# AshishKumar4/FlaxDiff

Measured on AMD Instinct MI355X. Metric: train images/sec/node (64x64 uncond EDM UNet, bs=256), higher is better.
Workload: dtype bf16; 1 GPU; model=unet_64px_[64,128,256,512]_res2_heads4, global_batch=256, resolution=64, parallelism=dp1, schedule=EDM + KarrasPredictionTransform(sigma_data=0.5)

## Files before the change

flaxdiff_amd/ops/hip/bindings.cpp:

```cpp
#include <torch/extension.h>
#include <tuple>
#include <vector>

std::vector<torch::Tensor> gn_silu_fwd(torch::Tensor x, torch::Tensor gamma,
                                       torch::Tensor beta, long groups,
                                       double eps, bool silu,
                                       c10::optional<torch::Tensor> x_b);
std::vector<torch::Tensor> gn_silu_bwd(torch::Tensor dy, torch::Tensor x,
                                       torch::Tensor gamma, torch::Tensor beta,
                                       torch::Tensor mean, torch::Tensor rstd,
                                       long groups, bool silu,
                                       c10::optional<torch::Tensor> dgamma_sink,
                                       c10::optional<torch::Tensor> dbeta_sink,
                                       c10::optional<torch::Tensor> add,
                                       c10::optional<torch::Tensor> x_b);
std::vector<torch::Tensor> rms_norm_fwd(torch::Tensor x, torch::Tensor gamma,
                                        double eps);
std::vector<torch::Tensor> rms_norm_bwd(torch::Tensor dy, torch::Tensor x,
                                        torch::Tensor gamma, torch::Tensor rrms,
                                        c10::optional<torch::Tensor> dgamma_sink);
torch::Tensor conv2d_fwd(torch::Tensor x, torch::Tensor w, torch::Tensor bias,
                         long stride, torch::Tensor add, torch::Tensor badd);
torch::Tensor conv2d_fwd_up2x(torch::Tensor x, torch::Tensor w,
                              torch::Tensor bias);
// ... 18 lines not shown
                                            torch::Tensor lse, double scale);
std::vector<torch::Tensor> attn_bwd_smallkv_v2(torch::Tensor q, torch::Tensor k,
                                               torch::Tensor v, torch::Tensor dout,
                                               torch::Tensor lse, double scale);
std::vector<torch::Tensor> attn_bwd_stream(torch::Tensor q, torch::Tensor k,
                                           torch::Tensor v, torch::Tensor o,
                                           torch::Tensor dout, torch::Tensor lse,
                                           double scale);
std::vector<int64_t> attn_bwd_stream_geometry(int64_t D);
torch::Tensor fwd_diffusion(torch::Tensor x0, torch::Tensor eps,
                            torch::Tensor a, torch::Tensor s);
torch::Tensor upsample2x_fwd(torch::Tensor x);
torch::Tensor time_embed(torch::Tensor t, torch::Tensor freqs, long features,
                         double max_positions);
torch::Tensor upsample2x_bwd(torch::Tensor dy);
torch::Tensor colsum(torch::Tensor x, c10::optional<torch::Tensor> sink);
torch::Tensor cat2_lastdim(torch::Tensor a, torch::Tensor b);
std::vector<torch::Tensor> split2_lastdim(torch::Tensor dy, long Ca, long Cb);
torch::Tensor geglu_fwd(torch::Tensor h);
torch::Tensor geglu_bwd(torch::Tensor dy, torch::Tensor h);
torch::Tensor wl2_loss_fwd(torch::Tensor pred, torch::Tensor target,
                           torch::Tensor wb);
torch::Tensor wl2_loss_bwd(torch::Tensor pred, torch::Tensor target,
                           torch::Tensor wb, torch::Tensor go);
torch::Tensor s5_scan_fwd(torch::Tensor a, torch::Tensor bu);
std::vector<torch::Tensor> s5_scan_bwd(torch::Tensor a, torch::Tensor x,
                                       torch::Tensor dx);
torch::Tensor gemm_fwd(torch::Tensor x, torch::Tensor w, torch::Tensor bias);
torch::Tensor gemm_dx(torch::Tensor dy, torch::Tensor w);
torch::Tensor gemm_nt(torch::Tensor x, torch::Tensor wt, torch::Tensor bias,
// ... 37 lines not shown
    m.def("attn_fwd", &attn_fwd, "flash attention forward (bf16, fp32 softmax)");
    m.def("attn_bwd_smallkv", &attn_bwd_smallkv,
          "fused attention backward for Skv<=128, D<=32");
    m.def("attn_bwd_smallkv_v2", &attn_bwd_smallkv_v2,
          "vectorized-LDS attention backward for Skv<=128, D<=64");
    m.def("attn_bwd_stream", &attn_bwd_stream,
          "key-streaming attention backward for any Sq/Skv, D<=128",
          py::arg("q"), py::arg("k"), py::arg("v"), py::arg("o"),
          py::arg("dout"), py::arg("lse"), py::arg("scale"));
    m.def("attn_bwd_stream_geometry", &attn_bwd_stream_geometry,
          "(DP, KB, QS) of attn_bwd_stream at head dim D");
    m.def("fwd_diffusion", &fwd_diffusion, "forward-diffusion axpy");
    m.def("upsample2x_fwd", &upsample2x_fwd, "nearest 2x upsample");
    m.def("time_embed", &time_embed, "fused sinusoidal/Fourier time embedding");
    m.def("upsample2x_bwd", &upsample2x_bwd, "nearest 2x upsample backward");
    m.def("colsum", &colsum, "coalesced column sum (bias grads)",
          py::arg("x"), py::arg("sink") = py::none());
    m.def("cat2_lastdim", &cat2_lastdim, "fused last-dim 2-tensor concat");
    m.def("split2_lastdim", &split2_lastdim, "one-pass last-dim split (cat backward)");
    m.def("geglu_fwd", &geglu_fwd, "fused GEGLU forward");
    m.def("geglu_bwd", &geglu_bwd, "fused GEGLU backward");
    m.def("wl2_loss_fwd", &wl2_loss_fwd, "fused weighted L2 loss forward");
    m.def("wl2_loss_bwd", &wl2_loss_bwd, "fused weighted L2 loss backward");
    m.def("s5_scan_fwd", &s5_scan_fwd, "S5 diagonal scan forward");
    m.def("s5_scan_bwd", &s5_scan_bwd, "S5 diagonal scan backward");
    m.def("gemm_fwd", &gemm_fwd, "MFMA bf16 GEMM y = x@w (+bias)");
    m.def("gemm_dx", &gemm_dx, "MFMA bf16 GEMM dx = dy@w^T");
    m.def("gemm_nt", &gemm_nt, "MFMA bf16 GEMM y = x@wt^T (+bias)",
          py::arg("x"), py::arg("wt"), py::arg("bias"), py::arg("add"),
          py::arg("x2") = py::none());
// ... 5 lines not shown
```

flaxdiff_amd/ops/hip/common.h:

```cpp
#pragma once

#include <hip/hip_runtime.h>
#include <hip/hip_bf16.h>
#include <hip/hip_fp16.h>
#include <cstdint>
#include <cstdlib>

#define FD_WAVE 64

__device__ __forceinline__ float bf2f(ushort u) {
    union { uint32_t i; float f; } c;
    c.i = uint32_t(u) << 16;
    return c.f;
}

__device__ __forceinline__ ushort f2bf(float f) {
    union { float f; uint32_t i; } c;
    c.f = f;
    uint32_t x = c.i;
    uint32_t lsb = (x >> 16) & 1;
    x += 0x7fff + lsb;
    return ushort(x >> 16);
}

typedef ushort ushort8 __attribute__((ext_vector_type(8)));
typedef float float8 __attribute__((ext_vector_type(8)));
typedef short bf16x8 __attribute__((ext_vector_type(8)));
typedef short bf16x4 __attribute__((ext_vector_type(4)));
typedef float f32x4 __attribute__((ext_vector_type(4)));
typedef float f32x16 __attribute__((ext_vector_type(16)));

struct BF16Tag {};
struct F32Tag {};

template <typename T> struct ElemIO;
template <> struct ElemIO<ushort> {
    static __device__ __forceinline__ float ld(const ushort* p) { return bf2f(*p); }
// ... 108 lines not shown
```

flaxdiff_amd/ops/hip/elementwise.hip:

```cpp
#include <torch/extension.h>
#include <ATen/hip/HIPContext.h>
#include "common.h"
#include "host_util.h"

template <typename T>
__global__ void fwd_diffusion_kernel(const T* __restrict__ x0,
                                     const T* __restrict__ eps,
                                     const float* __restrict__ a,
                                     const float* __restrict__ s,
                                     T* __restrict__ y,
                                     long per_sample, long total) {
    long i0 = (long)(blockIdx.x) * blockDim.x + threadIdx.x;
    const long stride = (long)gridDim.x * blockDim.x;
    for (long i = i0; i < total; i += stride) {
        const long b = i / per_sample;
        const float av = a[b], sv = s[b];
        ElemIO<T>::st(y + i, av * ElemIO<T>::ld(x0 + i) + sv * ElemIO<T>::ld(eps + i));
    }
}

template <typename T>
__global__ void upsample2x_fwd_kernel(const T* __restrict__ x, T* __restrict__ y,
                                      int H, int W, int C, long total_out) {
    long i0 = (long)(blockIdx.x) * blockDim.x + threadIdx.x;
// ... 139 lines not shown
    auto out = torch::empty({B, F}, tf.options());
    const float* fptr = nullptr;
    torch::Tensor ff;
    if (freqs.defined() && freqs.numel()) {
        ff = freqs.to(at::kFloat).contiguous();
        fptr = ff.data_ptr<float>();
    }
    const long total = (long)B * (F / 2);
    auto stream = at::hip::getCurrentHIPStream();
    hipLaunchKernelGGL(time_embed_kernel,
                       dim3((unsigned)((total + 255) / 256)), dim3(256), 0,
                       stream, tf.data_ptr<float>(), fptr,
                       out.data_ptr<float>(), B, F, (float)max_positions);
    FD_CHECK_LAUNCH();
    return out;
}


union GNV8_E { uint4 q; ushort u[8]; };

__global__ void colsum_kernel(const ushort* __restrict__ x,
                              float* __restrict__ out,
                              const long M, const int C,
                              const int rows_per_block) {
    extern __shared__ float csm[];
    const long r0 = (long)blockIdx.x * rows_per_block;
    const long r1 = min(r0 + rows_per_block, M);
    const int tpr = C >> 3;
    const int nsub = blockDim.x / tpr;
    for (int c = threadIdx.x; c < C; c += blockDim.x) csm[c] = 0.f;
// ... 338 lines not shown
```

flaxdiff_amd/ops/hip/gn_silu.hip:

```cpp
#include <torch/extension.h>
#include <ATen/hip/HIPContext.h>
#include "common.h"
#include "host_util.h"

template <typename T, bool SILU>
__global__ void gn_silu_fwd_kernel(const T* __restrict__ x,
                                   const float* __restrict__ gamma,
                                   const float* __restrict__ beta,
                                   T* __restrict__ y,
                                   float* __restrict__ mean_out,
                                   float* __restrict__ rstd_out,
                                   int S, int C, int G, float eps) {
    const int b = blockIdx.x / G;
    const int g = blockIdx.x % G;
    const int Cg = C / G;
    const long base = (long)b * S * C + (long)g * Cg;
    const long n = (long)S * Cg;

    __shared__ float scratch[4];

    float s1 = 0.f, s2 = 0.f;
    for (long i = threadIdx.x; i < n; i += blockDim.x) {
        const int s = i / Cg, c = i % Cg;
        const float v = ElemIO<T>::ld(x + base + (long)s * C + c);
// ... 90 lines not shown
            float dxv = rstd * (dz * gam - (s1 + xn * s2) * inv_n);
            if (HAS_ADD) dxv += ElemIO<T>::ld(add + idx);
            ElemIO<T>::st(dx + idx, dxv);
        }
        atomicAdd(dg_loc + c, dg_p);
        atomicAdd(db_loc + c, db_p);
    }

    __syncthreads();
    for (int cc = threadIdx.x; cc < Cg; cc += blockDim.x) {
        atomicAdd(dgamma + g * Cg + cc, dg_loc[cc]);
        atomicAdd(dbeta + g * Cg + cc, db_loc[cc]);
    }
}

union GNV8 { uint4 q; ushort u[8]; };



#define GN3_NTH 256

template <bool DUAL, typename P>
__device__ __forceinline__ P* gn3_src(P* xa, P* xb, const long row,
                                      const int c8, const int C, const int Ca) {
    if (DUAL)
        return c8 < Ca ? xa + row * Ca + c8 : xb + row * (C - Ca) + (c8 - Ca);
    return xa + row * C + c8;
}

template <bool SILU, bool DUAL = false>
__global__ void gn3_fwd_stats_kernel(const ushort* __restrict__ x,
                                     float* __restrict__ sums,
                                     const int S, const int C, const int G,
                                     const int Cg, const int chunk_rows,
                                     const FastDiv fdCg,
                                     const ushort* __restrict__ xb,
                                     const int Ca) {
    extern __shared__ float sm[];
    const int b = blockIdx.x;
    const int s0 = blockIdx.y * chunk_rows;
    const int s1lim = min(s0 + chunk_rows, S);
    const int tpr = C >> 3;
    const int nsub = GN3_NTH / tpr;
    const bool active = (int)threadIdx.x < nsub * tpr && nsub > 0;
    const int c8 = (threadIdx.x % tpr) * 8;
    const int srow = threadIdx.x / tpr;
    for (int i = threadIdx.x; i < 2 * G; i += GN3_NTH) sm[i] = 0.f;
    __syncthreads();

    float a1 = 0.f, a2 = 0.f;
    if (active) {
        for (int s = s0 + srow; s < s1lim; s += nsub) {
            GNV8 pk;
            pk.q = *reinterpret_cast<const uint4*>(
                gn3_src<DUAL>(x, xb, (long)b * S + s, c8, C, Ca));
            #pragma unroll
            for (int j = 0; j < 8; ++j) {
                const float v = bf2f(pk.u[j]);
                a1 += v; a2 += v * v;
            }
        }
        const int g = (int)fd_div((unsigned)c8, fdCg);
        atomicAdd(sm + g * 2 + 0, a1);
        atomicAdd(sm + g * 2 + 1, a2);
    }
    __syncthreads();
    for (int i = threadIdx.x; i < 2 * G; i += GN3_NTH)
        if (sm[i] != 0.f) atomicAdd(sums + (long)b * 2 * G + i, sm[i]);
}

template <bool SILU, bool DUAL = false>
__global__ void gn3_fwd_apply_kernel(const ushort* __restrict__ x,
                                     const float* __restrict__ sums,
                                     const float* __restrict__ gamma,
                                     const float* __restrict__ beta,
                                     ushort* __restrict__ y,
                                     float* __restrict__ mean_out,
                                     float* __restrict__ rstd_out,
                                     const int S, const int C, const int G,
                                     const int Cg, const int chunk_rows,
                                     const float eps, const FastDiv fdCg,
                                     const ushort* __restrict__ xb,
                                     const int Ca) {
    extern __shared__ float sm[];
    float* mr = sm;
    float* gam = sm + 2 * G;
    float* bet = gam + C;
    const int b = blockIdx.x;
    const int s0 = blockIdx.y * chunk_rows;
    const int s1lim = min(s0 + chunk_rows, S);
    const long base = ((long)b * S + s0) * C;
    const long n = (long)(s1lim - s0) * C;
    const float inv_n = 1.f / ((long)S * Cg);
    for (int g = threadIdx.x; g < G; g += GN3_NTH) {
        const float m = sums[(long)b * 2 * G + g * 2 + 0] * inv_n;
        const float var = fmaxf(sums[(long)b * 2 * G + g * 2 + 1] * inv_n - m * m, 0.f);
        mr[g * 2 + 0] = m;
        mr[g * 2 + 1] = rsqrtf(var + eps);
        if (blockIdx.y == 0) {
            mean_out[(long)b * G + g] = m;
            rstd_out[(long)b * G + g] = mr[g * 2 + 1];
        }
    }
    for (int c = threadIdx.x; c < C; c += GN3_NTH) {
        gam[c] = gamma[c];
        bet[c] = beta[c];
    }
    __syncthreads();

    unsigned cc = (unsigned)((threadIdx.x * 8) % C);
    const unsigned cstep = (unsigned)((GN3_NTH * 8) % C);
    long row = (long)b * S + s0 + (threadIdx.x * 8) / C;
    const int rstep = (GN3_NTH * 8) / C;
    for (long i = (long)threadIdx.x * 8; i < n; i += GN3_NTH * 8) {
        const unsigned c0 = cc;
        const long row0 = row;
        cc += cstep; if (cc >= (unsigned)C) cc -= C;
        if (DUAL) { row += rstep; if (cc < c0 + cstep) ++row; }
        const int g = (int)fd_div(c0, fdCg);
        const float m = mr[g * 2 + 0], r = mr[g * 2 + 1];
        GNV8 pk, out;
        pk.q = *reinterpret_cast<const uint4*>(
            DUAL ? gn3_src<true>(x, xb, row0, (int)c0, C, Ca) : x + base + i);
        #pragma unroll
        for (int j = 0; j < 8; ++j) {
            float z = (bf2f(pk.u[j]) - m) * r * gam[c0 + j] + bet[c0 + j];
            if (SILU) z = z / (1.f + __expf(-z));
            out.u[j] = f2bf(z);
        }
        *reinterpret_cast<uint4*>(y + base + i) = out.q;
    }
}

template <bool SILU, bool DUAL = false>
__global__ void gn3_bwd_stats_kernel(const ushort* __restrict__ dy,
                                     const ushort* __restrict__ x,
                                     const float* __restrict__ gamma,
                                     const float* __restrict__ beta,
                                     const float* __restrict__ mean_in,
                                     const float* __restrict__ rstd_in,
                                     float* __restrict__ gsums,
                                     float* __restrict__ dgamma,
                                     float* __restrict__ dbeta,
                                     const int S, const int C, const int G,
                                     const int Cg, const int chunk_rows,
                                     const FastDiv fdCg,
                                     const ushort* __restrict__ xb,
                                     const int Ca) {
    extern __shared__ float sm[];
    float* ss = sm;
    float* dgl = ss + 2 * G;
    float* dbl = dgl + C;
    const int b = blockIdx.x;
    const int s0 = blockIdx.y * chunk_rows;
    const int s1lim = min(s0 + chunk_rows, S);
    const int tpr = C >> 3;
    const int nsub = GN3_NTH / tpr;
    const bool active = (int)threadIdx.x < nsub * tpr && nsub > 0;
    const int c8 = (threadIdx.x % tpr) * 8;
    const int srow = threadIdx.x / tpr;
    for (int i = threadIdx.x; i < 2 * G; i += GN3_NTH) ss[i] = 0.f;
    for (int c = threadIdx.x; c < C; c += GN3_NTH) { dgl[c] = 0.f; dbl[c] = 0.f; }
    __syncthreads();

    if (active) {
        const int g = (int)fd_div((unsigned)c8, fdCg);
        const float m = mean_in[(long)b * G + g];
        const float r = rstd_in[(long)b * G + g];
        float g8[8], b8[8], dg8[8] = {}, db8[8] = {};
        #pragma unroll
        for (int j = 0; j < 8; ++j) {
            g8[j] = gamma[c8 + j];
            b8[j] = SILU ? beta[c8 + j] : 0.f;
        }
        float a1 = 0.f, a2 = 0.f;
        for (int s = s0 + srow; s < s1lim; s += nsub) {
            const long idx = ((long)b * S + s) * C + c8;
            GNV8 xv, dv;
            xv.q = *reinterpret_cast<const uint4*>(
                DUAL ? gn3_src<true>(x, xb, (long)b * S + s, c8, C, Ca)
                     : x + idx);
            dv.q = *reinterpret_cast<const uint4*>(dy + idx);
            #pragma unroll
            for (int j = 0; j < 8; ++j) {
                const float xn = (bf2f(xv.u[j]) - m) * r;
                float dz = bf2f(dv.u[j]);
                if (SILU) {
                    const float z = xn * g8[j] + b8[j];
                    const float sig = 1.f / (1.f + __expf(-z));
                    dz *= sig * (1.f + z * (1.f - sig));
                }
                dg8[j] += dz * xn;
                db8[j] += dz;
                const float dzg = dz * g8[j];
                a1 += dzg;
                a2 += dzg * xn;
            }
        }
        atomicAdd(ss + g * 2 + 0, a1);
        atomicAdd(ss + g * 2 + 1, a2);
        #pragma unroll
        for (int j = 0; j < 8; ++j) {
            atomicAdd(dgl + c8 + j, dg8[j]);
            atomicAdd(dbl + c8 + j, db8[j]);
        }
    }
    __syncthreads();
    for (int i = threadIdx.x; i < 2 * G; i += GN3_NTH)
        if (ss[i] != 0.f) atomicAdd(gsums + (long)b * 2 * G + i, ss[i]);
    for (int c = threadIdx.x; c < C; c += GN3_NTH) {
        if (dgl[c] != 0.f) atomicAdd(dgamma + c, dgl[c]);
        if (dbl[c] != 0.f) atomicAdd(dbeta + c, dbl[c]);
    }
}

template <bool SILU, bool HAS_ADD, bool DUAL = false>
__global__ void gn3_bwd_apply_kernel(const ushort* __restrict__ dy,
                                     const ushort* __restrict__ x,
                                     const float* __restrict__ gamma,
                                     const float* __restrict__ beta,
                                     const float* __restrict__ mean_in,
                                     const float* __restrict__ rstd_in,
                                     const float* __restrict__ gsums,
                                     const ushort* __restrict__ add,
                                     ushort* __restrict__ dx,
                                     const int S, const int C, const int G,
                                     const int Cg, const int chunk_rows,
                                     const FastDiv fdCg,
                                     const ushort* __restrict__ xb,
                                     ushort* __restrict__ dxb,
                                     const int Ca) {
    extern __shared__ float sm[];
    float* mrs = sm;
    float* gam = sm + 4 * G;
    float* bet = gam + C;
    const int b = blockIdx.x;
    const int s0 = blockIdx.y * chunk_rows;
    const int s1lim = min(s0 + chunk_rows, S);
    const long base = ((long)b * S + s0) * C;
    const long n = (long)(s1lim - s0) * C;
    for (int g = threadIdx.x; g < G; g += GN3_NTH) {
        mrs[g * 4 + 0] = mean_in[(long)b * G + g];
        mrs[g * 4 + 1] = rstd_in[(long)b * G + g];
        mrs[g * 4 + 2] = gsums[(long)b * 2 * G + g * 2 + 0];
        mrs[g * 4 + 3] = gsums[(long)b * 2 * G + g * 2 + 1];
    }
    for (int c = threadIdx.x; c < C; c += GN3_NTH) {
        gam[c] = gamma[c];
        bet[c] = SILU ? beta[c] : 0.f;
    }
    __syncthreads();
    const float inv_n = 1.f / ((long)S * Cg);

    unsigned cc = (unsigned)((threadIdx.x * 8) % C);
    const unsigned cstep = (unsigned)((GN3_NTH * 8) % C);
    long row = (long)b * S + s0 + (threadIdx.x * 8) / C;
    const int rstep = (GN3_NTH * 8) / C;
    for (long i = (long)threadIdx.x * 8; i < n; i += GN3_NTH * 8) {
        const unsigned c0 = cc;
        const long row0 = row;
        cc += cstep; if (cc >= (unsigned)C) cc -= C;
        if (DUAL) { row += rstep; if (cc < c0 + cstep) ++row; }
        const int g = (int)fd_div(c0, fdCg);
        const float m = mrs[g * 4 + 0], r = mrs[g * 4 + 1];
        const float s1 = mrs[g * 4 + 2], s2 = mrs[g * 4 + 3];
        GNV8 xv, dv, av, out;
        xv.q = *reinterpret_cast<const uint4*>(
            DUAL ? gn3_src<true>(x, xb, row0, (int)c0, C, Ca) : x + base + i);
        dv.q = *reinterpret_cast<const uint4*>(dy + base + i);
        if (HAS_ADD) av.q = *reinterpret_cast<const uint4*>(add + base + i);
        #pragma unroll
        for (int j = 0; j < 8; ++j) {
            const float xn = (bf2f(xv.u[j]) - m) * r;
            float dz = bf2f(dv.u[j]);
            if (SILU) {
                const float z = xn * gam[c0 + j] + bet[c0 + j];
                const float sig = 1.f / (1.f + __expf(-z));
                dz *= sig * (1.f + z * (1.f - sig));
            }
            float dxv = r * (dz * gam[c0 + j] - (s1 + xn * s2) * inv_n);
            if (HAS_ADD) dxv += bf2f(av.u[j]);
            out.u[j] = f2bf(dxv);
        }
        *reinterpret_cast<uint4*>(
            DUAL ? gn3_src<true>(dx, dxb, row0, (int)c0, C, Ca)
                 : dx + base + i) = out.q;
    }
}


static int gn_dual_check(const torch::Tensor& x,
                         const c10::optional<torch::Tensor>& x_b, long groups,
                         const char* who) {
    if (!fd_has(x_b)) return 0;
    const int Ca = x.size(-1), Cb = x_b->size(-1);
    const int C = Ca + Cb;
    TORCH_CHECK(x_b->is_cuda() && x_b->device() == x.device() &&
                x_b->is_contiguous() && x.is_contiguous() &&
                x_b->dim() == x.dim() &&
                x_b->sizes().slice(0, x.dim() - 1) ==
                    x.sizes().slice(0, x.dim() - 1),
                who, ": x_b must be contiguous with x's leading dims");
    TORCH_CHECK(x.scalar_type() == at::kBFloat16 &&
                x_b->scalar_type() == at::kBFloat16 && Ca % 8 == 0 &&
// ... 26 lines not shown
    auto f32opt = x.options().dtype(at::kFloat);
    auto mean = torch::empty({(long)B * G}, f32opt);
    auto rstd = torch::empty({(long)B * G}, f32opt);
    auto gamma_f = gamma.to(at::kFloat).contiguous();
    auto beta_f = beta.to(at::kFloat).contiguous();
    auto stream = at::hip::getCurrentHIPStream();
    dim3 grid(B * G), block(256);

    const int Cg_f = C / G;
    #define LAUNCH_FWD(T, SILU_) \
        hipLaunchKernelGGL((gn_silu_fwd_kernel<T, SILU_>), grid, block, 0, stream, \
            (const T*)x.data_ptr(), gamma_f.data_ptr<float>(), beta_f.data_ptr<float>(), \
            (T*)y.data_ptr(), mean.data_ptr<float>(), rstd.data_ptr<float>(), \
            (int)S, C, G, (float)eps)
    if (x.scalar_type() == at::kBFloat16 && Cg_f % 8 == 0 && C <= 2048) {
        auto sums = torch::zeros({(long)B * 2 * G}, f32opt);
        const int chunk_rows = std::max(1, 32768 / C);
        dim3 g3(B, (S + chunk_rows - 1) / chunk_rows);
        const FastDiv fdCg = make_fastdiv(Cg_f);
        #define L_STATS(SILU_, DUAL_)                                          \
            hipLaunchKernelGGL((gn3_fwd_stats_kernel<SILU_, DUAL_>),           \
                g3, dim3(GN3_NTH), 2 * G * sizeof(float), stream,              \
                (const ushort*)x.data_ptr(), sums.data_ptr<float>(),           \
                (int)S, C, G, Cg_f, chunk_rows, fdCg, xb_p, Ca)
        #define L_APPLY(SILU_, DUAL_)                                          \
            hipLaunchKernelGGL((gn3_fwd_apply_kernel<SILU_, DUAL_>),           \
                g3, dim3(GN3_NTH), (2 * G + 2 * C) * sizeof(float), stream,    \
                (const ushort*)x.data_ptr(), sums.data_ptr<float>(),           \
                gamma_f.data_ptr<float>(), beta_f.data_ptr<float>(),           \
                (ushort*)y.data_ptr(), mean.data_ptr<float>(),                 \
                rstd.data_ptr<float>(), (int)S, C, G, Cg_f, chunk_rows,        \
                (float)eps, fdCg, xb_p, Ca)
        if (dual) {
            if (silu) { L_STATS(true, true); L_APPLY(true, true); }
            else { L_STATS(false, true); L_APPLY(false, true); }
        } else {
            if (silu) { L_STATS(true, false); L_APPLY(true, false); }
            else { L_STATS(false, false); L_APPLY(false, false); }
        }
        #undef L_STATS
        #undef L_APPLY
    } else if (x.scalar_type() == at::kBFloat16) {
        if (silu) LAUNCH_FWD(ushort, true); else LAUNCH_FWD(ushort, false);
    } else {
        if (silu) LAUNCH_FWD(float, true); else LAUNCH_FWD(float, false);
    }
    #undef LAUNCH_FWD
    FD_CHECK_LAUNCH();
    return {y, mean, rstd};
}

std::vector<torch::Tensor> gn_silu_bwd(torch::Tensor dy, torch::Tensor x,
                                       torch::Tensor gamma, torch::Tensor beta,
// ... 26 lines not shown

    const bool has_add = fd_has(add);
    if (has_add)
        TORCH_CHECK(add->is_cuda() && add->device() == x.device() &&
                    add->is_contiguous() && add->sizes() == dy.sizes() &&
                    add->scalar_type() == x.scalar_type(),
                    "gn_silu_bwd: add must be a contiguous tensor of x's "
                    "shape, dtype and device");
    const void* add_p = has_add ? add->data_ptr() : nullptr;

    auto dx = torch::empty_like(x);
    torch::Tensor dxb;
    if (dual) dxb = torch::empty_like(*x_b);
    ushort* dxb_p = dual ? (ushort*)dxb.data_ptr() : nullptr;
    auto f32opt = x.options().dtype(at::kFloat);
    const long ngs = 2L * x.size(0) * G;
    auto zflat = torch::zeros({(has_sink ? 0L : 2L * C) + ngs}, f32opt);
    auto dgamma = has_sink ? *dgamma_sink : zflat.narrow(0, 0, C);
    auto dbeta = has_sink ? *dbeta_sink : zflat.narrow(0, C, C);
    auto gamma_f = gamma.to(at::kFloat).contiguous();
    auto beta_f = beta.to(at::kFloat).contiguous();
    auto stream = at::hip::getCurrentHIPStream();
    dim3 grid(B * G), block(256);
    const size_t smem = (2 * Cg + 4) * sizeof(float);

    #define LAUNCH_BWD_(T, SILU_, ADD_) \
        hipLaunchKernelGGL((gn_silu_bwd_kernel<T, SILU_, ADD_>), grid, block, smem, stream, \
            (const T*)dy.data_ptr(), (const T*)x.data_ptr(), gamma_f.data_ptr<float>(), \
            beta_f.data_ptr<float>(), mean.data_ptr<float>(), rstd.data_ptr<float>(), \
            (T*)dx.data_ptr(), dgamma.data_ptr<float>(), dbeta.data_ptr<float>(), \
            (const T*)add_p, (int)S, C, G)
    #define LAUNCH_BWD(T, SILU_) \
        do { if (has_add) LAUNCH_BWD_(T, SILU_, true); \
             else LAUNCH_BWD_(T, SILU_, false); } while (0)
    if (x.scalar_type() == at::kBFloat16 && Cg % 8 == 0 && C <= 2048) {
        auto gsums = zflat.narrow(0, has_sink ? 0L : 2L * C, ngs);
        static const long btarget = std::getenv("FD_GN_BLOCKS")
            ? atol(std::getenv("FD_GN_BLOCKS")) : 768L;
        const long bwant = std::max(1L, btarget / std::max(1, B));
        const int chunk_rows = std::max((int)((S + bwant - 1) / bwant),
                                        std::max(1, 32768 / C));
        dim3 g3(B, ((int)S + chunk_rows - 1) / chunk_rows);
        const FastDiv fdCg = make_fastdiv(Cg);
        #define L_BSTATS(SILU_, DUAL_)                                         \
            hipLaunchKernelGGL((gn3_bwd_stats_kernel<SILU_, DUAL_>),           \
                g3, dim3(GN3_NTH), (4 * G + 4 * C) * sizeof(float), stream,    \
                (const ushort*)dy.data_ptr(), (const ushort*)x.data_ptr(),     \
                gamma_f.data_ptr<float>(), beta_f.data_ptr<float>(),           \
                mean.data_ptr<float>(), rstd.data_ptr<float>(),                \
                gsums.data_ptr<float>(), dgamma.data_ptr<float>(),             \
                dbeta.data_ptr<float>(), (int)S, C, G, Cg, chunk_rows, fdCg,   \
                xb_p, Ca)
        #define L_BAPPLY(SILU_, ADD_, DUAL_)                                   \
            hipLaunchKernelGGL((gn3_bwd_apply_kernel<SILU_, ADD_, DUAL_>),     \
                g3, dim3(GN3_NTH), (4 * G + 2 * C) * sizeof(float), stream,    \
                (const ushort*)dy.data_ptr(), (const ushort*)x.data_ptr(),     \
                gamma_f.data_ptr<float>(), beta_f.data_ptr<float>(),           \
                mean.data_ptr<float>(), rstd.data_ptr<float>(),                \
                gsums.data_ptr<float>(), (const ushort*)add_p,                 \
                (ushort*)dx.data_ptr(), (int)S, C, G, Cg, chunk_rows, fdCg,    \
                xb_p, dxb_p, Ca)
        #define L_BWD3(SILU_, DUAL_)                                           \
            do { L_BSTATS(SILU_, DUAL_);                                       \
                 if (has_add) L_BAPPLY(SILU_, true, DUAL_);                    \
                 else L_BAPPLY(SILU_, false, DUAL_); } while (0)
        if (dual) {
            if (silu) L_BWD3(true, true); else L_BWD3(false, true);
        } else {
            if (silu) L_BWD3(true, false); else L_BWD3(false, false);
        }
        #undef L_BWD3
        #undef L_BSTATS
        #undef L_BAPPLY
    } else if (x.scalar_type() == at::kBFloat16) {
// ... 15 lines not shown
```

Baseline: 6113 images/s.

## Restructure GroupNorm-SiLU kernels with per-thread column mapping and partial-sum chunks

Rewrites the bf16 GroupNorm(+SiLU) forward and backward stats/apply kernels. Each thread now owns a fixed 8-channel column and walks rows with a 4-way unrolled load loop. Per-group statistics are written as per-chunk partials through an LDS tree and summed by the apply kernel, which replaces the global atomics and the zero-initialised buffers. The block size is chosen from C so every thread is active, packed bf16 conversion uses a vector builtin, and SiLU uses a fast reciprocal. This removes atomics, zero-fill launches and LDS staging of gamma/beta, at the cost of redundant chunk-sum reads in the apply kernels and slightly different rounding and accuracy behaviour.

```diff
diff --git a/flaxdiff_amd/ops/hip/bindings.cpp b/flaxdiff_amd/ops/hip/bindings.cpp
--- a/flaxdiff_amd/ops/hip/bindings.cpp
+++ b/flaxdiff_amd/ops/hip/bindings.cpp
@@ -56,6 +56,7 @@
 torch::Tensor time_embed(torch::Tensor t, torch::Tensor freqs, long features,
                          double max_positions);
 torch::Tensor upsample2x_bwd(torch::Tensor dy);
+torch::Tensor bf16_round_rne(torch::Tensor x);
 torch::Tensor colsum(torch::Tensor x, c10::optional<torch::Tensor> sink);
 torch::Tensor cat2_lastdim(torch::Tensor a, torch::Tensor b);
 std::vector<torch::Tensor> split2_lastdim(torch::Tensor dy, long Ca, long Cb);
@@ -123,6 +124,8 @@
     m.def("upsample2x_fwd", &upsample2x_fwd, "nearest 2x upsample");
     m.def("time_embed", &time_embed, "fused sinusoidal/Fourier time embedding");
     m.def("upsample2x_bwd", &upsample2x_bwd, "nearest 2x upsample backward");
+    m.def("bf16_round_rne", &bf16_round_rne,
+          "fp32 -> bf16 through f2bf_pk (round-to-nearest-even)");
     m.def("colsum", &colsum, "coalesced column sum (bias grads)",
           py::arg("x"), py::arg("sink") = py::none());
     m.def("cat2_lastdim", &cat2_lastdim, "fused last-dim 2-tensor concat");
diff --git a/flaxdiff_amd/ops/hip/common.h b/flaxdiff_amd/ops/hip/common.h
--- a/flaxdiff_amd/ops/hip/common.h
+++ b/flaxdiff_amd/ops/hip/common.h
@@ -21,6 +21,14 @@
     uint32_t lsb = (x >> 16) & 1;
     x += 0x7fff + lsb;
     return ushort(x >> 16);
+}
+
+__device__ __forceinline__ uint32_t f2bf_pk(float lo, float hi) {
+    typedef float f2bf_f32x2 __attribute__((ext_vector_type(2)));
+    typedef __bf16 f2bf_bf16x2 __attribute__((ext_vector_type(2)));
+    union { f2bf_bf16x2 v; uint32_t u; } c;
+    c.v = __builtin_convertvector(f2bf_f32x2{lo, hi}, f2bf_bf16x2);
+    return c.u;
 }
 
 typedef ushort ushort8 __attribute__((ext_vector_type(8)));
diff --git a/flaxdiff_amd/ops/hip/elementwise.hip b/flaxdiff_amd/ops/hip/elementwise.hip
--- a/flaxdiff_amd/ops/hip/elementwise.hip
+++ b/flaxdiff_amd/ops/hip/elementwise.hip
@@ -177,6 +177,32 @@
                        out.data_ptr<float>(), B, F, (float)max_positions);
     FD_CHECK_LAUNCH();
     return out;
+}
+
+
+__global__ void bf16_round_rne_kernel(const float2* __restrict__ x,
+                                      uint32_t* __restrict__ y, const long n2) {
+    const long stride = (long)gridDim.x * blockDim.x;
+    for (long i = (long)blockIdx.x * blockDim.x + threadIdx.x; i < n2;
+         i += stride) {
+        const float2 v = x[i];
+        y[i] = f2bf_pk(v.x, v.y);
+    }
+}
+
+torch::Tensor bf16_round_rne(torch::Tensor x) {
+    FD_FLUSH_STALE();
+    TORCH_CHECK(x.is_cuda() && x.is_contiguous() &&
+                x.scalar_type() == at::kFloat && x.numel() % 2 == 0,
+                "bf16_round_rne: contiguous fp32 tensor of even length");
+    auto y = torch::empty(x.sizes(), x.options().dtype(at::kBFloat16));
+    const long n2 = x.numel() / 2;
+    auto stream = at::hip::getCurrentHIPStream();
+    hipLaunchKernelGGL(bf16_round_rne_kernel, dim3(grid_1d(n2, 256)), dim3(256),
+                       0, stream, (const float2*)x.data_ptr(),
+                       (uint32_t*)y.data_ptr(), n2);
+    FD_CHECK_LAUNCH();
+    return y;
 }
 
 
diff --git a/flaxdiff_amd/ops/hip/gn_silu.hip b/flaxdiff_amd/ops/hip/gn_silu.hip
--- a/flaxdiff_amd/ops/hip/gn_silu.hip
+++ b/flaxdiff_amd/ops/hip/gn_silu.hip
@@ -128,280 +128,399 @@
     }
 }
 
-union GNV8 { uint4 q; ushort u[8]; };
-
-
-
-#define GN3_NTH 256
+
+
+#define GN3_MAX_NTH 640
+#define GN3_U 4
+
+struct Gn3Map {
+    int tpr, nsub;
+    int srow, c8;
+    bool active;
+};
+
+__device__ __forceinline__ Gn3Map gn3_map(const int C) {
+    Gn3Map t;
+    t.tpr = C >> 3;
+    t.nsub = blockDim.x / t.tpr;
+    t.srow = threadIdx.x / t.tpr;
+    t.c8 = (threadIdx.x - t.srow * t.tpr) * 8;
+    t.active = t.srow < t.nsub;
+    return t;
+}
 
 template <bool DUAL, typename P>
-__device__ __forceinline__ P* gn3_src(P* xa, P* xb, const long row,
-                                      const int c8, const int C, const int Ca) {
-    if (DUAL)
-        return c8 < Ca ? xa + row * Ca + c8 : xb + row * (C - Ca) + (c8 - Ca);
-    return xa + row * C + c8;
-}
-
-template <bool SILU, bool DUAL = false>
-__global__ void gn3_fwd_stats_kernel(const ushort* __restrict__ x,
-                                     float* __restrict__ sums,
-                                     const int S, const int C, const int G,
-                                     const int Cg, const int chunk_rows,
-                                     const FastDiv fdCg,
-                                     const ushort* __restrict__ xb,
-                                     const int Ca) {
+__device__ __forceinline__ P* gn3_col(P* a, P* b, const int c8, const int C,
+                                      const int Ca, int& stride) {
+    if (DUAL) {
+        if (c8 < Ca) { stride = Ca; return a + c8; }
+        stride = C - Ca;
+        return b + (c8 - Ca);
+    }
+    stride = C;
+    return a + c8;
+}
+
+__device__ __forceinline__ void gn3_unpack(const uint4 q, float (&v)[8]) {
+    const uint32_t w[4] = {q.x, q.y, q.z, q.w};
+    #pragma unroll
+    for (int j = 0; j < 4; ++j) {
+        v[2 * j] = __uint_as_float(w[j] << 16);
+        v[2 * j + 1] = __uint_as_float(w[j] & 0xffff0000u);
+    }
+}
+
+__device__ __forceinline__ uint4 gn3_pack(const float (&v)[8]) {
+    return make_uint4(f2bf_pk(v[0], v[1]), f2bf_pk(v[2], v[3]),
+                      f2bf_pk(v[4], v[5]), f2bf_pk(v[6], v[7]));
+}
+
+__device__ __forceinline__ float gn3_sigmoid(const float z) {
+    return __builtin_amdgcn_rcpf(1.f + __expf(-z));
+}
+
+template <bool SILU>
+__device__ __forceinline__ float gn3_dz(const float dy, const float tc,
+                                        const float rg, const float bt) {
+    if (!SILU) return dy;
+    const float z = fmaf(tc, rg, bt);
+    const float sig = gn3_sigmoid(z);
+    return dy * (sig * fmaf(z, 1.f - sig, 1.f));
+}
+
+__device__ __forceinline__ void gn3_block_group_sums(
+        const float a1, const float a2, const Gn3Map& t, float* sm,
+        float* __restrict__ out, const int G, const int opg) {
+    float* tv = sm;
+    float* slot = sm + 2 * blockDim.x;
+    if (t.active)
+        *reinterpret_cast<float2*>(tv + 2 * threadIdx.x) = make_float2(a1, a2);
+    __syncthreads();
+    for (int i = threadIdx.x; i < 2 * G * t.nsub; i += blockDim.x) {
+        const int sg = i >> 1;
+        const int r = sg / G, g = sg - r * G;
+        const float* p = tv + 2 * (r * t.tpr + g * opg) + (i & 1);
+        float acc = 0.f;
+        for (int o = 0; o < opg; ++o) acc += p[2 * o];
+        slot[i] = acc;
+    }
+    __syncthreads();
+    for (int i = threadIdx.x; i < 2 * G; i += blockDim.x) {
+        float acc = 0.f;
+        for (int r = 0; r < t.nsub; ++r) acc += slot[r * 2 * G + i];
+        out[i] = acc;
+    }
+}
+
+__device__ __forceinline__ float2 gn3_sum_chunks(const float* __restrict__ part,
+                                                 const int b, const int g,
+                                                 const int G) {
+    const float* p = part + ((long)b * gridDim.y * G + g) * 2;
+    float2 acc = make_float2(0.f, 0.f);
+    for (int k = 0; k < (int)gridDim.y; ++k, p += 2 * G) {
+        const float2 v = *reinterpret_cast<const float2*>(p);
+        acc.x += v.x; acc.y += v.y;
+    }
+    return acc;
+}
+
+template <bool DUAL>
+__global__ __launch_bounds__(GN3_MAX_NTH)
+void gn3_fwd_stats_kernel(const ushort* __restrict__ x,
+                          float* __restrict__ part,
+                          const int S, const int C, const int G, const int Cg,
+                          const int chunk_rows,
+                          const ushort* __restrict__ xb, const int Ca) {
     extern __shared__ float sm[];
+    const Gn3Map t = gn3_map(C);
     const int b = blockIdx.x;
     const int s0 = blockIdx.y * chunk_rows;
     const int s1lim = min(s0 + chunk_rows, S);
-    const int tpr = C >> 3;
-    const int nsub = GN3_NTH / tpr;
-    const bool active = (int)threadIdx.x < nsub * tpr && nsub > 0;
-    const int c8 = (threadIdx.x % tpr) * 8;
-    const int srow = threadIdx.x / tpr;
-    for (int i = threadIdx.x; i < 2 * G; i += GN3_NTH) sm[i] = 0.f;
-    __syncthreads();
 
     float a1 = 0.f, a2 = 0.f;
-    if (active) {
-        for (int s = s0 + srow; s < s1lim; s += nsub) {
-            GNV8 pk;
-            pk.q = *reinterpret_cast<const uint4*>(
-                gn3_src<DUAL>(x, xb, (long)b * S + s, c8, C, Ca));
+    if (t.active) {
+        int stride;
+        const ushort* p = gn3_col<DUAL>(x, xb, t.c8, C, Ca, stride);
+        const long step = (long)t.nsub * stride;
+        int s = s0 + t.srow;
+        p += ((long)b * S + s) * stride;
+        for (; s + (GN3_U - 1) * t.nsub < s1lim;
+             s += GN3_U * t.nsub, p += GN3_U * step) {
+            uint4 q[GN3_U];
+            #pragma unroll
+            for (int u = 0; u < GN3_U; ++u)
+                q[u] = *reinterpret_cast<const uint4*>(p + u * step);
+            #pragma unroll
+            for (int u = 0; u < GN3_U; ++u) {
+                float v[8];
+                gn3_unpack(q[u], v);
+                #pragma unroll
+                for (int j = 0; j < 8; ++j) {
+                    a1 += v[j]; a2 = fmaf(v[j], v[j], a2);
+                }
+            }
+        }
+        for (; s < s1lim; s += t.nsub, p += step) {
+            float v[8];
+            gn3_unpack(*reinterpret_cast<const uint4*>(p), v);
             #pragma unroll
             for (int j = 0; j < 8; ++j) {
-                const float v = bf2f(pk.u[j]);
-                a1 += v; a2 += v * v;
+                a1 += v[j]; a2 = fmaf(v[j], v[j], a2);
             }
         }
-        const int g = (int)fd_div((unsigned)c8, fdCg);
-        atomicAdd(sm + g * 2 + 0, a1);
-        atomicAdd(sm + g * 2 + 1, a2);
-    }
-    __syncthreads();
-    for (int i = threadIdx.x; i < 2 * G; i += GN3_NTH)
-        if (sm[i] != 0.f) atomicAdd(sums + (long)b * 2 * G + i, sm[i]);
-}
-
-template <bool SILU, bool DUAL = false>
-__global__ void gn3_fwd_apply_kernel(const ushort* __restrict__ x,
-                                     const float* __restrict__ sums,
-                                     const float* __restrict__ gamma,
-                                     const float* __restrict__ beta,
-                                     ushort* __restrict__ y,
-                                     float* __restrict__ mean_out,
-                                     float* __restrict__ rstd_out,
-                                     const int S, const int C, const int G,
-                                     const int Cg, const int chunk_rows,
-                                     const float eps, const FastDiv fdCg,
-                                     const ushort* __restrict__ xb,
-                                     const int Ca) {
-    extern __shared__ float sm[];
-    float* mr = sm;
-    float* gam = sm + 2 * G;
-    float* bet = gam + C;
+    }
+    gn3_block_group_sums(a1, a2, t, sm,
+                         part + ((long)b * gridDim.y + blockIdx.y) * 2 * G,
+                         G, Cg >> 3);
+}
+
+template <bool SILU>
+__device__ __forceinline__ uint4 gn3_fwd_octet(const uint4 q, const float m,
+                                               const float (&sc)[8],
+                                               const float (&bt)[8]) {
+    float v[8];
+    gn3_unpack(q, v);
+    #pragma unroll
+    for (int j = 0; j < 8; ++j) {
+        const float z = fmaf(v[j] - m, sc[j], bt[j]);
+        v[j] = SILU ? z * gn3_sigmoid(z) : z;
+    }
+    return gn3_pack(v);
+}
+
+template <bool SILU, bool DUAL>
+__global__ __launch_bounds__(GN3_MAX_NTH)
+void gn3_fwd_apply_kernel(const ushort* __restrict__ x,
+                          const float* __restrict__ part,
+                          const float* __restrict__ gamma,
+                          const float* __restrict__ beta,
+                          ushort* __restrict__ y,
+                          float* __restrict__ mean_out,
+                          float* __restrict__ rstd_out,
+                          const int S, const int C, const int G, const int Cg,
+                          const int chunk_rows, const float eps,
+                          const FastDiv fdCg,
+                          const ushort* __restrict__ xb, const int Ca) {
+    const Gn3Map t = gn3_map(C);
+    if (!t.active) return;
     const int b = blockIdx.x;
     const int s0 = blockIdx.y * chunk_rows;
     const int s1lim = min(s0 + chunk_rows, S);
-    const long base = ((long)b * S + s0) * C;
-    const long n = (long)(s1lim - s0) * C;
+    const int g = (int)fd_div((unsigned)t.c8, fdCg);
+
+    const float2 tot = gn3_sum_chunks(part, b, g, G);
     const float inv_n = 1.f / ((long)S * Cg);
-    for (int g = threadIdx.x; g < G; g += GN3_NTH) {
-        const float m = sums[(long)b * 2 * G + g * 2 + 0] * inv_n;
-        const float var = fmaxf(sums[(long)b * 2 * G + g * 2 + 1] * inv_n - m * m, 0.f);
-        mr[g * 2 + 0] = m;
-        mr[g * 2 + 1] = rsqrtf(var + eps);
-        if (blockIdx.y == 0) {
-            mean_out[(long)b * G + g] = m;
-            rstd_out[(long)b * G + g] = mr[g * 2 + 1];
-        }
-    }
-    for (int c = threadIdx.x; c < C; c += GN3_NTH) {
-        gam[c] = gamma[c];
-        bet[c] = beta[c];
-    }
-    __syncthreads();
-
-    unsigned cc = (unsigned)((threadIdx.x * 8) % C);
-    const unsigned cstep = (unsigned)((GN3_NTH * 8) % C);
-    long row = (long)b * S + s0 + (threadIdx.x * 8) / C;
-    const int rstep = (GN3_NTH * 8) / C;
-    for (long i = (long)threadIdx.x * 8; i < n; i += GN3_NTH * 8) {
-        const unsigned c0 = cc;
-        const long row0 = row;
-        cc += cstep; if (cc >= (unsigned)C) cc -= C;
-        if (DUAL) { row += rstep; if (cc < c0 + cstep) ++row; }
-        const int g = (int)fd_div(c0, fdCg);
-        const float m = mr[g * 2 + 0], r = mr[g * 2 + 1];
-        GNV8 pk, out;
-        pk.q = *reinterpret_cast<const uint4*>(
-            DUAL ? gn3_src<true>(x, xb, row0, (int)c0, C, Ca) : x + base + i);
+    const float m = tot.x * inv_n;
+    const float r = rsqrtf(fmaxf(tot.y * inv_n - m * m, 0.f) + eps);
+    if (blockIdx.y == 0 && t.srow == 0 && t.c8 == g * Cg) {
+        mean_out[(long)b * G + g] = m;
+        rstd_out[(long)b * G + g] = r;
+    }
+    float sc[8], bt[8];
+    #pragma unroll
+    for (int j = 0; j < 8; ++j) {
+        sc[j] = r * gamma[t.c8 + j];
+        bt[j] = beta[t.c8 + j];
+    }
+
+    int stride;
+    const ushort* p = gn3_col<DUAL>(x, xb, t.c8, C, Ca, stride);
+    const long step = (long)t.nsub * stride, ystep = (long)t.nsub * C;
+    int s = s0 + t.srow;
+    p += ((long)b * S + s) * stride;
+    ushort* py = y + ((long)b * S + s) * C + t.c8;
+    for (; s + (GN3_U - 1) * t.nsub < s1lim;
+         s += GN3_U * t.nsub, p += GN3_U * step, py += GN3_U * ystep) {
+        uint4 q[GN3_U];
         #pragma unroll
-        for (int j = 0; j < 8; ++j) {
-            float z = (bf2f(pk.u[j]) - m) * r * gam[c0 + j] + bet[c0 + j];
-            if (SILU) z = z / (1.f + __expf(-z));
-            out.u[j] = f2bf(z);
-        }
-        *reinterpret_cast<uint4*>(y + base + i) = out.q;
-    }
-}
-
-template <bool SILU, bool DUAL = false>
-__global__ void gn3_bwd_stats_kernel(const ushort* __restrict__ dy,
-                                     const ushort* __restrict__ x,
-                                     const float* __restrict__ gamma,
-                                     const float* __restrict__ beta,
-                                     const float* __restrict__ mean_in,
-                                     const float* __restrict__ rstd_in,
-                                     float* __restrict__ gsums,
-                                     float* __restrict__ dgamma,
-                                     float* __restrict__ dbeta,
-                                     const int S, const int C, const int G,
-                                     const int Cg, const int chunk_rows,
-                                     const FastDiv fdCg,
-                                     const ushort* __restrict__ xb,
-                                     const int Ca) {
+        for (int u = 0; u < GN3_U; ++u)
+            q[u] = *reinterpret_cast<const uint4*>(p + u * step);
+        #pragma unroll
+        for (int u = 0; u < GN3_U; ++u)
+            q[u] = gn3_fwd_octet<SILU>(q[u], m, sc, bt);
+        #pragma unroll
+        for (int u = 0; u < GN3_U; ++u)
+            *reinterpret_cast<uint4*>(py + u * ystep) = q[u];
+    }
+    for (; s < s1lim; s += t.nsub, p += step, py += ystep)
+        *reinterpret_cast<uint4*>(py) = gn3_fwd_octet<SILU>(
+            *reinterpret_cast<const uint4*>(p), m, sc, bt);
+}
+
+template <bool SILU>
+__device__ __forceinline__ void gn3_bstats_octet(const uint4 xq, const uint4 dq,
+                                                 const float m,
+                                                 const float (&rg)[8],
+                                                 const float (&bt)[8],
+                                                 float (&dg)[8],
+                                                 float (&db)[8]) {
+    float xv[8], dv[8];
+    gn3_unpack(xq, xv);
+    gn3_unpack(dq, dv);
+    #pragma unroll
+    for (int j = 0; j < 8; ++j) {
+        const float tc = xv[j] - m;
+        const float dz = gn3_dz<SILU>(dv[j], tc, rg[j], bt[j]);
+        dg[j] = fmaf(dz, tc, dg[j]);
+        db[j] += dz;
+    }
+}
+
+template <bool SILU, bool DUAL>
+__global__ __launch_bounds__(GN3_MAX_NTH)
+void gn3_bwd_stats_kernel(const ushort* __restrict__ dy,
+                          const ushort* __restrict__ x,
+                          const float* __restrict__ gamma,
+                          const float* __restrict__ beta,
+                          const float* __restrict__ mean_in,
+                          const float* __restrict__ rstd_in,
+                          float* __restrict__ part,
+                          float* __restrict__ dgamma,
+                          float* __restrict__ dbeta,
+                          const int S, const int C, const int G, const int Cg,
+                          const int chunk_rows, const FastDiv fdCg,
+                          const ushort* __restrict__ xb, const int Ca) {
     extern __shared__ float sm[];
-    float* ss = sm;
-    float* dgl = ss + 2 * G;
+    float* dgl = sm;
     float* dbl = dgl + C;
+    const Gn3Map t = gn3_map(C);
     const int b = blockIdx.x;
     const int s0 = blockIdx.y * chunk_rows;
     const int s1lim = min(s0 + chunk_rows, S);
-    const int tpr = C >> 3;
-    const int nsub = GN3_NTH / tpr;
-    const bool active = (int)threadIdx.x < nsub * tpr && nsub > 0;
-    const int c8 = (threadIdx.x % tpr) * 8;
-    const int srow = threadIdx.x / tpr;
-    for (int i = threadIdx.x; i < 2 * G; i += GN3_NTH) ss[i] = 0.f;
-    for (int c = threadIdx.x; c < C; c += GN3_NTH) { dgl[c] = 0.f; dbl[c] = 0.f; }
+    for (int c = threadIdx.x; c < 2 * C; c += blockDim.x) sm[c] = 0.f;
     __syncthreads();
 
-    if (active) {
-        const int g = (int)fd_div((unsigned)c8, fdCg);
+    float a1 = 0.f, a2 = 0.f;
+    if (t.active) {
+        const int g = (int)fd_div((unsigned)t.c8, fdCg);
         const float m = mean_in[(long)b * G + g];
         const float r = rstd_in[(long)b * G + g];
-        float g8[8], b8[8], dg8[8] = {}, db8[8] = {};
+        float rg[8], bt[8], dg[8] = {}, db[8] = {};
         #pragma unroll
         for (int j = 0; j < 8; ++j) {
-            g8[j] = gamma[c8 + j];
-            b8[j] = SILU ? beta[c8 + j] : 0.f;
+            rg[j] = r * gamma[t.c8 + j];
+            bt[j] = SILU ? beta[t.c8 + j] : 0.f;
         }
-        float a1 = 0.f, a2 = 0.f;
-        for (int s = s0 + srow; s < s1lim; s += nsub) {
-            const long idx = ((long)b * S + s) * C + c8;
-            GNV8 xv, dv;
-            xv.q = *reinterpret_cast<const uint4*>(
-                DUAL ? gn3_src<true>(x, xb, (long)b * S + s, c8, C, Ca)
-                     : x + idx);
-            dv.q = *reinterpret_cast<const uint4*>(dy + idx);
-            #pragma unroll
-            for (int j = 0; j < 8; ++j) {
-                const float xn = (bf2f(xv.u[j]) - m) * r;
-                float dz = bf2f(dv.u[j]);
-                if (SILU) {
-                    const float z = xn * g8[j] + b8[j];
-                    const float sig = 1.f / (1.f + __expf(-z));
-                    dz *= sig * (1.f + z * (1.f - sig));
-                }
-                dg8[j] += dz * xn;
-                db8[j] += dz;
-                const float dzg = dz * g8[j];
-                a1 += dzg;
-                a2 += dzg * xn;
-            }
-        }
-        atomicAdd(ss + g * 2 + 0, a1);
-        atomicAdd(ss + g * 2 + 1, a2);
+        int stride;
+        const ushort* p = gn3_col<DUAL>(x, xb, t.c8, C, Ca, stride);
+        const long step = (long)t.nsub * stride, dstep = (long)t.nsub * C;
+        int s = s0 + t.srow;
+        p += ((long)b * S + s) * stride;
+        const ushort* pd = dy + ((long)b * S + s) * C + t.c8;
+        for (; s < s1lim; s += t.nsub, p += step, pd += dstep)
+            gn3_bstats_octet<SILU>(*reinterpret_cast<const uint4*>(p),
+                                   *reinterpret_cast<const uint4*>(pd),
+                                   m, rg, bt, dg, db);
         #pragma unroll
         for (int j = 0; j < 8; ++j) {
-            atomicAdd(dgl + c8 + j, dg8[j]);
-            atomicAdd(dbl + c8 + j, db8[j]);
+            dg[j] *= r;
+            const float gam = gamma[t.c8 + j];
+            a1 = fmaf(gam, db[j], a1);
+            a2 = fmaf(gam, dg[j], a2);
+            atomicAdd(dgl + t.c8 + j, dg[j]);
+            atomicAdd(dbl + t.c8 + j, db[j]);
         }
     }
-    __syncthreads();
-    for (int i = threadIdx.x; i < 2 * G; i += GN3_NTH)
-        if (ss[i] != 0.f) atomicAdd(gsums + (long)b * 2 * G + i, ss[i]);
-    for (int c = threadIdx.x; c < C; c += GN3_NTH) {
+    gn3_block_group_sums(a1, a2, t, sm + 2 * C,
+                         part + ((long)b * gridDim.y + blockIdx.y) * 2 * G,
+                         G, Cg >> 3);
+    for (int c = threadIdx.x; c < C; c += blockDim.x) {
         if (dgl[c] != 0.f) atomicAdd(dgamma + c, dgl[c]);
         if (dbl[c] != 0.f) atomicAdd(dbeta + c, dbl[c]);
     }
 }
 
-template <bool SILU, bool HAS_ADD, bool DUAL = false>
-__global__ void gn3_bwd_apply_kernel(const ushort* __restrict__ dy,
-                                     const ushort* __restrict__ x,
-                                     const float* __restrict__ gamma,
-                                     const float* __restrict__ beta,
-                                     const float* __restrict__ mean_in,
-                                     const float* __restrict__ rstd_in,
-                                     const float* __restrict__ gsums,
-                                     const ushort* __restrict__ add,
-                                     ushort* __restrict__ dx,
-                                     const int S, const int C, const int G,
-                                     const int Cg, const int chunk_rows,
-                                     const FastDiv fdCg,
-                                     const ushort* __restrict__ xb,
-                                     ushort* __restrict__ dxb,
-                                     const int Ca) {
-    extern __shared__ float sm[];
-    float* mrs = sm;
-    float* gam = sm + 4 * G;
-    float* bet = gam + C;
+template <bool SILU, bool HAS_ADD>
+__device__ __forceinline__ uint4 gn3_bapply_octet(const uint4 xq, const uint4 dq,
+                                                  const uint4 aq, const float m,
+                                                  const float (&rg)[8],
+                                                  const float (&bt)[8],
+                                                  const float nk1,
+                                                  const float nk2) {
+    float xv[8], dv[8], av[8];
+    gn3_unpack(xq, xv);
+    gn3_unpack(dq, dv);
+    if (HAS_ADD) gn3_unpack(aq, av);
+    #pragma unroll
+    for (int j = 0; j < 8; ++j) {
+        const float tc = xv[j] - m;
+        const float dz = gn3_dz<SILU>(dv[j], tc, rg[j], bt[j]);
+        const float dxv = fmaf(dz, rg[j], fmaf(tc, nk2, nk1));
+        xv[j] = HAS_ADD ? dxv + av[j] : dxv;
+    }
+    return gn3_pack(xv);
+}
+
+template <bool SILU, bool HAS_ADD, bool DUAL>
+__global__ __launch_bounds__(GN3_MAX_NTH)
+void gn3_bwd_apply_kernel(const ushort* __restrict__ dy,
+                          const ushort* __restrict__ x,
+                          const float* __restrict__ gamma,
+                          const float* __restrict__ beta,
+                          const float* __restrict__ mean_in,
+                          const float* __restrict__ rstd_in,
+                          const float* __restrict__ part,
+                          const ushort* __restrict__ add,
+                          ushort* __restrict__ dx,
+                          const int S, const int C, const int G, const int Cg,
+                          const int chunk_rows, const FastDiv fdCg,
+                          const ushort* __restrict__ xb,
+                          ushort* __restrict__ dxb, const int Ca) {
+    const Gn3Map t = gn3_map(C);
+    if (!t.active) return;
     const int b = blockIdx.x;
     const int s0 = blockIdx.y * chunk_rows;
     const int s1lim = min(s0 + chunk_rows, S);
-    const long base = ((long)b * S + s0) * C;
-    const long n = (long)(s1lim - s0) * C;
-    for (int g = threadIdx.x; g < G; g += GN3_NTH) {
-        mrs[g * 4 + 0] = mean_in[(long)b * G + g];
-        mrs[g * 4 + 1] = rstd_in[(long)b * G + g];
-        mrs[g * 4 + 2] = gsums[(long)b * 2 * G + g * 2 + 0];
-        mrs[g * 4 + 3] = gsums[(long)b * 2 * G + g * 2 + 1];
-    }
-    for (int c = threadIdx.x; c < C; c += GN3_NTH) {
-        gam[c] = gamma[c];
-        bet[c] = SILU ? beta[c] : 0.f;
-    }
-    __syncthreads();
-    const float inv_n = 1.f / ((long)S * Cg);
-
-    unsigned cc = (unsigned)((threadIdx.x * 8) % C);
-    const unsigned cstep = (unsigned)((GN3_NTH * 8) % C);
-    long row = (long)b * S + s0 + (threadIdx.x * 8) / C;
-    const int rstep = (GN3_NTH * 8) / C;
-    for (long i = (long)threadIdx.x * 8; i < n; i += GN3_NTH * 8) {
-        const unsigned c0 = cc;
-        const long row0 = row;
-        cc += cstep; if (cc >= (unsigned)C) cc -= C;
-        if (DUAL) { row += rstep; if (cc < c0 + cstep) ++row; }
-        const int g = (int)fd_div(c0, fdCg);
-        const float m = mrs[g * 4 + 0], r = mrs[g * 4 + 1];
-        const float s1 = mrs[g * 4 + 2], s2 = mrs[g * 4 + 3];
-        GNV8 xv, dv, av, out;
-        xv.q = *reinterpret_cast<const uint4*>(
-            DUAL ? gn3_src<true>(x, xb, row0, (int)c0, C, Ca) : x + base + i);
-        dv.q = *reinterpret_cast<const uint4*>(dy + base + i);
-        if (HAS_ADD) av.q = *reinterpret_cast<const uint4*>(add + base + i);
-        #pragma unroll
-        for (int j = 0; j < 8; ++j) {
-            const float xn = (bf2f(xv.u[j]) - m) * r;
-            float dz = bf2f(dv.u[j]);
-            if (SILU) {
-                const float z = xn * gam[c0 + j] + bet[c0 + j];
-                const float sig = 1.f / (1.f + __expf(-z));
-                dz *= sig * (1.f + z * (1.f - sig));
-            }
-            float dxv = r * (dz * gam[c0 + j] - (s1 + xn * s2) * inv_n);
-            if (HAS_ADD) dxv += bf2f(av.u[j]);
-            out.u[j] = f2bf(dxv);
-        }
-        *reinterpret_cast<uint4*>(
-            DUAL ? gn3_src<true>(dx, dxb, row0, (int)c0, C, Ca)
-                 : dx + base + i) = out.q;
-    }
-}
-
+    const int g = (int)fd_div((unsigned)t.c8, fdCg);
+    const float m = mean_in[(long)b * G + g];
+    const float r = rstd_in[(long)b * G + g];
+    const float2 tot = gn3_sum_chunks(part, b, g, G);
+    const float rn = r * (1.f / ((long)S * Cg));
+    const float nk1 = -rn * tot.x, nk2 = -rn * r * tot.y;
+    float rg[8], bt[8];
+    #pragma unroll
+    for (int j = 0; j < 8; ++j) {
+        rg[j] = r * gamma[t.c8 + j];
+        bt[j] = SILU ? beta[t.c8 + j] : 0.f;
+    }
+
+    int stride;
+    const ushort* p = gn3_col<DUAL>(x, xb, t.c8, C, Ca, stride);
+    ushort* po = gn3_col<DUAL>(dx, dxb, t.c8, C, Ca, stride);
+    const long step = (long)t.nsub * stride, dstep = (long)t.nsub * C;
+    int s = s0 + t.srow;
+    p += ((long)b * S + s) * stride;
+    po += ((long)b * S + s) * stride;
+    const long doff = ((long)b * S + s) * C + t.c8;
+    const ushort* pd = dy + doff;
+    const ushort* pa = HAS_ADD ? add + doff : nullptr;
+    for (; s < s1lim; s += t.nsub, p += step, po += step, pd += dstep,
+                      pa += HAS_ADD ? dstep : 0) {
+        uint4 aq = make_uint4(0, 0, 0, 0);
+        if (HAS_ADD) aq = *reinterpret_cast<const uint4*>(pa);
+        *reinterpret_cast<uint4*>(po) = gn3_bapply_octet<SILU, HAS_ADD>(
+            *reinterpret_cast<const uint4*>(p),
+            *reinterpret_cast<const uint4*>(pd), aq, m, rg, bt, nk1, nk2);
+    }
+}
+
+
+static int gn3_block(const int C) {
+    const int l = std::lcm(C / 8, 64);
+    const int nth = (256 + l - 1) / l * l;
+    return nth <= GN3_MAX_NTH ? nth : 256;
+}
+
+static int gn3_chunk_rows(const long S, const int B, const int C) {
+    static const long btarget = std::getenv("FD_GN_BLOCKS")
+        ? atol(std::getenv("FD_GN_BLOCKS")) : 768L;
+    const long bwant = std::max(1L, btarget / std::max(1, B));
+    return std::max((int)((S + bwant - 1) / bwant), std::max(1, 32768 / C));
+}
+
+static size_t gn3_sums_lds(const int nth, const int C, const int G) {
+    return (2 * nth + 2 * G * (nth / (C / 8))) * sizeof(float);
+}
 
 static int gn_dual_check(const torch::Tensor& x,
                          const c10::optional<torch::Tensor>& x_b, long groups,
@@ -458,29 +577,30 @@
             (T*)y.data_ptr(), mean.data_ptr<float>(), rstd.data_ptr<float>(), \
             (int)S, C, G, (float)eps)
     if (x.scalar_type() == at::kBFloat16 && Cg_f % 8 == 0 && C <= 2048) {
-        auto sums = torch::zeros({(long)B * 2 * G}, f32opt);
-        const int chunk_rows = std::max(1, 32768 / C);
-        dim3 g3(B, (S + chunk_rows - 1) / chunk_rows);
+        const int chunk_rows = gn3_chunk_rows(S, B, C);
+        const int nth = gn3_block(C);
+        dim3 g3(B, ((int)S + chunk_rows - 1) / chunk_rows);
+        auto part = torch::empty({(long)B * g3.y * G * 2}, f32opt);
         const FastDiv fdCg = make_fastdiv(Cg_f);
-        #define L_STATS(SILU_, DUAL_)                                          \
-            hipLaunchKernelGGL((gn3_fwd_stats_kernel<SILU_, DUAL_>),           \
-                g3, dim3(GN3_NTH), 2 * G * sizeof(float), stream,              \
-                (const ushort*)x.data_ptr(), sums.data_ptr<float>(),           \
-                (int)S, C, G, Cg_f, chunk_rows, fdCg, xb_p, Ca)
+        #define L_STATS(DUAL_)                                                 \
+            hipLaunchKernelGGL((gn3_fwd_stats_kernel<DUAL_>),                  \
+                g3, dim3(nth), gn3_sums_lds(nth, C, G), stream,                \
+                (const ushort*)x.data_ptr(), part.data_ptr<float>(),           \
+                (int)S, C, G, Cg_f, chunk_rows, xb_p, Ca)
         #define L_APPLY(SILU_, DUAL_)                                          \
             hipLaunchKernelGGL((gn3_fwd_apply_kernel<SILU_, DUAL_>),           \
-                g3, dim3(GN3_NTH), (2 * G + 2 * C) * sizeof(float), stream,    \
-                (const ushort*)x.data_ptr(), sums.data_ptr<float>(),           \
+                g3, dim3(nth), 0, stream,                                      \
+                (const ushort*)x.data_ptr(), part.data_ptr<float>(),           \
                 gamma_f.data_ptr<float>(), beta_f.data_ptr<float>(),           \
                 (ushort*)y.data_ptr(), mean.data_ptr<float>(),                 \
                 rstd.data_ptr<float>(), (int)S, C, G, Cg_f, chunk_rows,        \
                 (float)eps, fdCg, xb_p, Ca)
         if (dual) {
-            if (silu) { L_STATS(true, true); L_APPLY(true, true); }
-            else { L_STATS(false, true); L_APPLY(false, true); }
+            L_STATS(true);
+            if (silu) L_APPLY(true, true); else L_APPLY(false, true);
         } else {
-            if (silu) { L_STATS(true, false); L_APPLY(true, false); }
-            else { L_STATS(false, false); L_APPLY(false, false); }
+            L_STATS(false);
+            if (silu) L_APPLY(true, false); else L_APPLY(false, false);
         }
         #undef L_STATS
         #undef L_APPLY
@@ -537,8 +657,8 @@
     if (dual) dxb = torch::empty_like(*x_b);
     ushort* dxb_p = dual ? (ushort*)dxb.data_ptr() : nullptr;
     auto f32opt = x.options().dtype(at::kFloat);
-    const long ngs = 2L * x.size(0) * G;
-    auto zflat = torch::zeros({(has_sink ? 0L : 2L * C) + ngs}, f32opt);
+    torch::Tensor zflat;
+    if (!has_sink) zflat = torch::zeros({2L * C}, f32opt);
     auto dgamma = has_sink ? *dgamma_sink : zflat.narrow(0, 0, C);
     auto dbeta = has_sink ? *dbeta_sink : zflat.narrow(0, C, C);
     auto gamma_f = gamma.to(at::kFloat).contiguous();
@@ -557,30 +677,28 @@
         do { if (has_add) LAUNCH_BWD_(T, SILU_, true); \
              else LAUNCH_BWD_(T, SILU_, false); } while (0)
     if (x.scalar_type() == at::kBFloat16 && Cg % 8 == 0 && C <= 2048) {
-        auto gsums = zflat.narrow(0, has_sink ? 0L : 2L * C, ngs);
-        static const long btarget = std::getenv("FD_GN_BLOCKS")
-            ? atol(std::getenv("FD_GN_BLOCKS")) : 768L;
-        const long bwant = std::max(1L, btarget / std::max(1, B));
-        const int chunk_rows = std::max((int)((S + bwant - 1) / bwant),
-                                        std::max(1, 32768 / C));
+        const int chunk_rows = gn3_chunk_rows(S, B, C);
+        const int nth = gn3_block(C);
         dim3 g3(B, ((int)S + chunk_rows - 1) / chunk_rows);
+        auto part = torch::empty({(long)B * g3.y * G * 2}, f32opt);
         const FastDiv fdCg = make_fastdiv(Cg);
         #define L_BSTATS(SILU_, DUAL_)                                         \
             hipLaunchKernelGGL((gn3_bwd_stats_kernel<SILU_, DUAL_>),           \
-                g3, dim3(GN3_NTH), (4 * G + 4 * C) * sizeof(float), stream,    \
+                g3, dim3(nth),                                                 \
+                2 * C * sizeof(float) + gn3_sums_lds(nth, C, G), stream,       \
                 (const ushort*)dy.data_ptr(), (const ushort*)x.data_ptr(),     \
                 gamma_f.data_ptr<float>(), beta_f.data_ptr<float>(),           \
                 mean.data_ptr<float>(), rstd.data_ptr<float>(),                \
-                gsums.data_ptr<float>(), dgamma.data_ptr<float>(),             \
+                part.data_ptr<float>(), dgamma.data_ptr<float>(),              \
                 dbeta.data_ptr<float>(), (int)S, C, G, Cg, chunk_rows, fdCg,   \
                 xb_p, Ca)
         #define L_BAPPLY(SILU_, ADD_, DUAL_)                                   \
             hipLaunchKernelGGL((gn3_bwd_apply_kernel<SILU_, ADD_, DUAL_>),     \
-                g3, dim3(GN3_NTH), (4 * G + 2 * C) * sizeof(float), stream,    \
+                g3, dim3(nth), 0, stream,                                      \
                 (const ushort*)dy.data_ptr(), (const ushort*)x.data_ptr(),     \
                 gamma_f.data_ptr<float>(), beta_f.data_ptr<float>(),           \
                 mean.data_ptr<float>(), rstd.data_ptr<float>(),                \
-                gsums.data_ptr<float>(), (const ushort*)add_p,                 \
+                part.data_ptr<float>(), (const ushort*)add_p,                  \
                 (ushort*)dx.data_ptr(), (int)S, C, G, Cg, chunk_rows, fdCg,    \
                 xb_p, dxb_p, Ca)
         #define L_BWD3(SILU_, DUAL_)                                           \
```

After: 6259 images/s (median of 6 runs). 1.02x the previous value.
